# medvedevgroup/SibeliaZ

Hardware: AMD Instinct MI355X
Metric: seed vertices/sec through BlocksFinder (higher is better)
Workload: dtype int32

## Files before the change

### sibeliaz_amd/csrc/lcb_kernel.h

```cpp
#ifndef LCB_KERNEL_H
#define LCB_KERNEL_H

#include <hip/hip_runtime.h>
#include <stdint.h>

#include "lcb_kernel_limits.h"

#define LCB_EMPTY_KEY INT32_MIN
#if defined(__HIP_DEVICE_COMPILE__)
#define LCB_NO_LOADS_IN_FLIGHT() __builtin_amdgcn_s_waitcnt(0x0F70)
#else
#define LCB_NO_LOADS_IN_FLIGHT() ((void)0)
#endif
#if defined(__HIP_DEVICE_COMPILE__)
#define LCB_GLOBAL_U32(p) ((const __attribute__((address_space(1))) uint32_t*)(p))
#else
#define LCB_GLOBAL_U32(p) (p)
#endif
#ifndef LCB_PROF_PUSH
#define LCB_PROF_PUSH 0
#endif

template <int MODE> struct LcbCfg;
template <> struct LcbCfg<0> { static constexpr uint32_t IC = 256, VC = 1024, BW = 256, PC = 0; static constexpr bool INST_LDS = true, IDX_LDS = true; typedef uint16_t Idx; typedef uint32_t VLast; };
// ... 115 lines not shown

#define LCB_WAVE_SYNC_LDS()                                       \
    do {                                                          \
        __builtin_amdgcn_fence(__ATOMIC_RELEASE, "wavefront");    \
        __builtin_amdgcn_wave_barrier();                          \
        __builtin_amdgcn_fence(__ATOMIC_ACQUIRE, "wavefront");    \
    } while (0)
#define LCB_SYNC_IF(ldsResident) do { if (ldsResident) LCB_WAVE_SYNC_LDS(); else LCB_WAVE_SYNC(); } while (0)

#define LCB_MARK(S, slot, value)                                                         \
    do {                                                                                 \
        if ((S).dbg && (S).lane == 0) __hip_atomic_store(&(S).dbg[(slot)], (uint32_t)(value), __ATOMIC_RELAXED, __HIP_MEMORY_SCOPE_SYSTEM); \
    } while (0)

__device__ __forceinline__ uint32_t lcb_rfl(uint32_t v) { return (uint32_t)__builtin_amdgcn_readfirstlane((int)v); }
__device__ __forceinline__ int32_t lcb_rfl(int32_t v) { return __builtin_amdgcn_readfirstlane(v); }
__device__ __forceinline__ uint64_t lcb_rfl(uint64_t v) { return ((uint64_t)lcb_rfl((uint32_t)(v >> 32)) << 32) | lcb_rfl((uint32_t)v); }
__device__ __forceinline__ uint32_t lcb_rl(uint32_t v, uint32_t l) { return (uint32_t)__builtin_amdgcn_readlane((int)v, (int)l); }
__device__ __forceinline__ uint64_t lcb_rl(uint64_t v, uint32_t l) { return ((uint64_t)lcb_rl((uint32_t)(v >> 32), l) << 32) | lcb_rl((uint32_t)v, l); }
__device__ __forceinline__ int32_t lcb_rl(int32_t v, uint32_t l) { return __builtin_amdgcn_readlane(v, (int)l); }

__device__ __forceinline__ uint32_t lcb_wave_umax(uint32_t v)
{
    uint32_t t;
    t = (uint32_t)__builtin_amdgcn_update_dpp(0, (int)v, 0x111, 0xf, 0xf, false); v = v > t ? v : t;
    t = (uint32_t)__builtin_amdgcn_update_dpp(0, (int)v, 0x112, 0xf, 0xf, false); v = v > t ? v : t;
    t = (uint32_t)__builtin_amdgcn_update_dpp(0, (int)v, 0x114, 0xf, 0xf, false); v = v > t ? v : t;
    t = (uint32_t)__builtin_amdgcn_update_dpp(0, (int)v, 0x118, 0xf, 0xf, false); v = v > t ? v : t;
    t = (uint32_t)__builtin_amdgcn_update_dpp(0, (int)v, 0x142, 0xa, 0xf, false); v = v > t ? v : t;
    t = (uint32_t)__builtin_amdgcn_update_dpp(0, (int)v, 0x143, 0xc, 0xf, false); v = v > t ? v : t;
    return lcb_rl(v, 63);
}
__device__ __forceinline__ uint32_t lcb_wave_umin(uint32_t v) { return ~lcb_wave_umax(~v); }

#define LCB_FLAG_POS 1u
#define LCB_FLAG_BACKFIN 2u
#define LCB_FLAG_FRONTFIN 4u
#define LCB_FLAG_BITS 3u
#define LCB_FLAG_SEG_SHIFT (LCB_SEG_SHIFT + LCB_FLAG_BITS)

template <bool WIDE> struct LcbWidth { typedef uint32_t T; };
template <> struct LcbWidth<true> { typedef uint64_t T; };

template <int MODE_, bool SEG_>
struct LcbStateT {
    static constexpr int MODE = MODE_;
    typedef typename LcbCfg<MODE_>::Idx Idx;
    typedef typename LcbCfg<MODE_>::VLast VLast;
    static constexpr uint32_t NONE = (uint32_t)(Idx)~(Idx)0;
    static constexpr uint32_t LAST_SHIFT = 4u * sizeof(VLast);
    static constexpr bool SEG = SEG_;
    typedef typename LcbWidth<SEG_>::T Flat;
    typedef typename LcbWidth<SEG_>::T OccIdx;
    typedef uint32_t* FieldU;
    typedef int32_t* FieldI;
    LcbTables T;
    LcbUsed U;
    LcbKParams P;
    uint32_t lane;
    const uint64_t* segBase;
    uint32_t* segFirst;
    FieldU iFrontG, iBackG, iFrontPos, iBackPos, iLo, iHi, iFlags;
    FieldI iFrontDist, iBackDist;
    uint32_t* ordKey;
    Idx* ordIdx;
    Idx* good;
    Idx* goodPos;
    Idx* touch;
    uint32_t nTouch, nInit;
    uint32_t endInst;
    FieldU fpLo, fpHi;
    uint8_t* fpSeg8;
    uint32_t* fpSeg32;
    uint32_t nFp;
    uint32_t fpSplit, fpShift;
    uint32_t instCap;
    int32_t* vKey;
    uint32_t* vCount;
    VLast* vLast;
    Idx* vTouched;
    uint32_t* vNClaimed;
    uint32_t* vTicket;
    uint32_t* vOvf;
    uint32_t voteCap, voteShift;
    uint32_t* scr;
    uint32_t* bloom;
    uint32_t bloomShift;
    uint32_t* mail;
    uint32_t* part;
    unsigned long long* mailWalk;
    int32_t* pKeys;
    uint32_t* pSlots;
    uint32_t pathCap, pathShift;
    unsigned long long* body;
    uint32_t bodyCap;
    uint4* best;
    uint32_t bestCap;
    uint32_t* ck;
    uint32_t ckN, ckInst, ckGood, ckPath;
    int32_t ckFlank;
    uint32_t nInst, nGood, cur, nPath, nRight, nLeft, nBest, status;
    int32_t rightFlank, leftFlank;
    uint32_t* dbg;
    const uint32_t* abort;
    uint32_t pfPush, pfVote, pfMaxProbe, pfMaxInst;
    uint64_t pfTVote, pfTPush, pfTScore;
    uint64_t pfTWalk, pfTWaitB, pfTReduce, pfTScan;
    uint64_t pfVoters, pfChunks, pfTouchSum;
    uint64_t cWalk, cOcc, cCompatCall, cCompatStep, cVote, cPush;
};

#ifndef LCB_TEST_FP_SLOT_DIV
#define LCB_TEST_FP_SLOT_DIV 1u
#endif
template <class ST>
__device__ __forceinline__ uint32_t lcb_fp_slot(const ST& S, uint32_t i)
{
    if (i < S.fpSplit) return i;
    const uint32_t f = i + S.fpShift;
    return f < S.instCap / LCB_TEST_FP_SLOT_DIV ? f : i;
}

template <class ST>
__device__ __forceinline__ void lcb_fp_set_seg(ST& S, uint32_t fs, uint32_t seg)
{
    if (ST::SEG) { if (LcbCfg<ST::MODE>::INST_LDS) S.fpSeg8[fs] = (uint8_t)seg; else S.fpSeg32[fs] = seg; }
}
template <class ST>
__device__ __forceinline__ uint32_t lcb_fp_get_seg(const ST& S, uint32_t fs)
{
    return ST::SEG ? (LcbCfg<ST::MODE>::INST_LDS ? (uint32_t)S.fpSeg8[fs] : S.fpSeg32[fs]) : 0u;
}

enum { LCB_F_FRONTG = 0, LCB_F_BACKG, LCB_F_FRONTPOS, LCB_F_BACKPOS, LCB_F_LO, LCB_F_HI, LCB_F_FLAGS, LCB_F_FRONTDIST, LCB_F_BACKDIST, LCB_F_COUNT };
template <class ST>
__device__ __forceinline__ uint32_t lcb_inst_fields(const ST& S, uint32_t i)
{
    const uint32_t stride = (uint32_t)(S.iBackG - S.iFrontG);
    uint32_t f = 0;
    if (S.lane < (uint32_t)LCB_F_COUNT) f = S.iFrontG[S.lane * stride + i];
    return f;
}

__device__ __forceinline__ uint32_t lcb_hash(int32_t vid, uint32_t shift)
{
    return ((uint32_t)vid * 2654435761u) >> shift;
}

__device__ __forceinline__ LcbUsed lcb_used_of(const LcbTables& T, uint32_t view)
{
    LcbUsed U;
    U.live = T.used;
    U.tab = view ? T.viewTab + (size_t)view * T.nPages : nullptr;
    return U;
}

__device__ __forceinline__ uint32_t lcb_uword(const LcbUsed& U, uint32_t w)
{
    if (U.tab) w += LCB_GLOBAL_U32(U.tab)[w >> LCB_PAGE_SHIFT];
    return U.live[w];
}

template <class ST>
__device__ __forceinline__ typename ST::Flat lcb_seg_base(const ST& S, uint32_t seg) { return ST::SEG ? (typename ST::Flat)S.segBase[seg] : (typename ST::Flat)0; }
__device__ __forceinline__ uint32_t lcb_cw_seg(uint32_t cw) { return cw >> LCB_SEG_SHIFT; }
__device__ __forceinline__ uint32_t lcb_fl_seg(uint32_t fl) { return fl >> LCB_FLAG_SEG_SHIFT; }
// ... 477 lines not shown
                uint32_t first = 0;
#define LCB_SCAN64(x, base) if (!first && n > (base)) { const uint32_t c_ = n - (base) < 64u ? n - (base) : 64u; const uint64_t m_ = (x) & (c_ == 64u ? ~0ull : ((1ull << c_) - 1ull)); if (m_) first = (base) + (uint32_t)__ffsll((long long)m_); }
                LCB_SCAN64(x0, 0u) LCB_SCAN64(x1, 64u) LCB_SCAN64(x2, 128u) LCB_SCAN64(x3, 192u)
#undef LCB_SCAN64
                for (uint32_t d = have + 1; !first && d <= Lu; d++)
                    if (lcb_used_bit(S.U, (Flat)(up ? fb + (d - 1u) : fb - (d - 1u)))) first = d;
                if (first) { nv = first - 1u; brk = 1u; }
            }
        }
        if (isV && !tryUsed) {
            const uint32_t ge = up ? g0 + nv : g0 - nv;
            const uint32_t fs = lcb_fp_slot(S, vI);
            atomicMin(&S.fpLo[fs], ge);
            atomicMax(&S.fpHi[fs], ge);
        }
        if (STATS && isV) S.cWalk += nv + brk;
        auto consume = [&](uint32_t b, uint32_t c, int32_t id) {
            if (PROF) S.pfChunks++;
            const uint32_t bn = lcb_rl(nv, b), bf = lcb_rl(fl, b);
            const uint32_t d = c * 64 + S.lane + 1;
            bool act = d <= bn;
            const int32_t vid = (bf & LCB_FLAG_POS) ? id : -id;
            if (exact) {
                const unsigned long long hitM = __ballot(act && lcb_path_contains(S, vid));
                if (hitM) {
                    const uint32_t fh = (uint32_t)__ffsll((long long)hitM) - 1u;
                    act = act && S.lane < fh;
                    if (S.lane == b) {
                        const uint32_t nn = c * 64 + fh;
                        if (STATS) S.cWalk += (uint64_t)(nn + 1u) - (uint64_t)(nv + brk);
                        nv = nn; brk = 1u;
                    }
                }
            }
            const uint32_t wgt = lcb_rl(weight, b), e = lcb_rl(vE, b);
            if (act) {
                uint32_t h = lcb_hash(vid, S.voteShift);
                int32_t old = atomicCAS(&S.vKey[h], LCB_EMPTY_KEY, vid);
                uint32_t probe = 0;
                while (old != LCB_EMPTY_KEY && old != vid && probe < S.voteCap) {
                    h = (h + 1) & vmask; probe++;
                    old = atomicCAS(&S.vKey[h], LCB_EMPTY_KEY, vid);
                }
                if (old == LCB_EMPTY_KEY) {
                    const uint32_t tt = atomicAdd(S.vNClaimed, 1u);
                    if (tt < claimCap) S.vTouched[tt] = (typename ST::Idx)h; else *S.vOvf = 1u;
                }
                if (old == LCB_EMPTY_KEY || old == vid) {
                    atomicAdd(&S.vCount[h], wgt);
                    atomicMax(&S.vLast[h], ((typename ST::VLast)e << ST::LAST_SHIFT) | d);
                } else *S.vOvf = 1u;
            }
        };
        unsigned long long rest = walkM;
        uint32_t curB = 0, curC = 0, curN = 0, ord = 0;
        bool curOn = false;
        auto nextItem = [&](uint32_t& b, uint32_t& c) -> bool {
            for (;;) {
                if (curOn) {
                    curN = lcb_rl(nv, curB);
                    if (curC * 64 < curN) { b = curB; c = curC++; return true; }
                    curOn = false;
                }
                if (!rest) return false;
                curB = (uint32_t)__ffsll((long long)rest) - 1u; rest &= rest - 1;
                curC = ord < (uint32_t)LCB_VB ? 1u : 0u; ord++;
                curOn = true;
            }
        };
        for (;;) {
#pragma unroll
            for (int q = 0; q < LCB_VB; q++) if (itV[q]) consume(itB[q], itC[q], itId[q]);
#pragma unroll
            for (int q = 0; q < LCB_VB; q++) {
                itV[q] = nextItem(itB[q], itC[q]);
                itId[q] = 0;
                if (itV[q]) itId[q] = request(itB[q], itC[q]);
            }
            if (!itV[0]) break;
        }
    }
}

template <class ST>
__device__ inline bool lcb_vote_any_in_path(const ST& S, uint32_t s0, uint32_t s1)
{
    bool hit = false;
    for (uint32_t q = s0 + S.lane; q < s1; q += 64) if (lcb_path_contains(S, S.vKey[S.vTouched[q]])) hit = true;
    return __ballot(hit) != 0;
}

struct LcbBest { uint32_t cnt, keyHi, keyLo; int32_t vid; uint32_t e; };

template <class ST>
__device__ inline LcbBest lcb_vote_argmax(const ST& S, bool forward, bool useGood, uint32_t s0, uint32_t s1)
{
    uint32_t bCnt = 0, bHi = 0xFFFFFFFFu, bLo = 0xFFFFFFFFu, bE = 0;
    int32_t bVid = 0;
    for (uint32_t q = s0 + S.lane; q < s1; q += 64) {
        const uint32_t t = S.vTouched[q];
        const int32_t key = S.vKey[t];
        const uint32_t cnt = S.vCount[t];
        const typename ST::VLast last = S.vLast[t];
        const uint32_t e = (uint32_t)(last >> ST::LAST_SHIFT), d = (uint32_t)(last & (((typename ST::VLast)1 << ST::LAST_SHIFT) - 1));
        const uint32_t i = useGood ? S.good[e] : e;
        const uint32_t g0 = forward ? S.iBackG[i] : S.iFrontG[i];
        const uint32_t afl = S.iFlags[i];
        const uint32_t hi = ((afl & LCB_FLAG_POS) << 31) | (ST::SEG ? lcb_fl_seg(afl) << 26 : 0u) | (g0 >> 6), lo = (g0 << 26) | d;
        if (cnt > bCnt || (cnt == bCnt && (hi < bHi || (hi == bHi && lo < bLo)))) { bCnt = cnt; bHi = hi; bLo = lo; bVid = key; bE = e; }
    }
    LcbBest r;
    r.cnt = lcb_wave_umax(bCnt);
    bool c = bCnt == r.cnt && r.cnt != 0;
    r.keyHi = lcb_wave_umin(c ? bHi : 0xFFFFFFFFu);
    c = c && bHi == r.keyHi;
    r.keyLo = lcb_wave_umin(c ? bLo : 0xFFFFFFFFu);
    c = c && bLo == r.keyLo;
    const unsigned long long m = __ballot(c);
    const uint32_t w = m ? (uint32_t)__ffsll((long long)m) - 1u : 0u;
    r.vid = m ? lcb_rl(bVid, w) : 0;
    r.e = lcb_rl(bE, w);
    return r;
}

enum { LCB_MAIL_CMD = 0, LCB_MAIL_FLAGS, LCB_MAIL_NLIST, LCB_MAIL_FLANK, LCB_MAIL_NTOUCH, LCB_MAIL_FPSPLIT, LCB_MAIL_FPSHIFT, LCB_MAIL_WORDS = 8 };
enum { LCB_CMD_VOTE = 1, LCB_CMD_EXIT = 2 };

template <class ST>
__device__ inline void lcb_vote_clear(ST& S, uint32_t s0, uint32_t s1)
{
    for (uint32_t q = s0 + S.lane; q < s1; q += 64) { const uint32_t t = S.vTouched[q]; S.vKey[t] = LCB_EMPTY_KEY; S.vCount[t] = 0; S.vLast[t] = 0; }
}

#ifndef LCB_VOTE_SHARE_MIN
#define LCB_VOTE_SHARE_MIN 24u
#endif

template <int NW, class ST>
__device__ inline void lcb_vote_reduce_slice(ST& S, bool forward, bool useGood, uint32_t waveId, uint32_t nTouched, bool exact)
{
    const uint32_t per = (nTouched + NW - 1) / NW;
    const uint32_t s0 = waveId * per < nTouched ? waveId * per : nTouched, s1 = s0 + per < nTouched ? s0 + per : nTouched;
    const bool hit = !exact && lcb_vote_any_in_path(S, s0, s1);
    const LcbBest b = lcb_vote_argmax(S, forward, useGood, s0, s1);
    if (S.lane == 0) {
        uint32_t* p = S.part + 8 * waveId;
        p[0] = b.cnt; p[1] = b.keyHi; p[2] = b.keyLo; p[3] = (uint32_t)b.vid; p[4] = b.e; p[5] = hit ? 1u : 0u;
    }
    __syncthreads();
    lcb_vote_clear(S, s0, s1);
    __syncthreads();
}

template <bool STATS, int NW, bool PROF = false, class ST>
__device__ inline LcbBest lcb_vote_pass(ST& S, bool forward, bool tryUsed, bool useGood, bool exact, bool& ovfAny, bool& hit)
{
    const uint32_t claimCap = S.voteCap - (S.voteCap >> 2);
    LcbBest b;
    hit = false;
    const bool multi = NW > 1 && S.nTouch > 1;
    const bool share = multi && S.nTouch >= LCB_VOTE_SHARE_MIN;
    if (multi) {
        if (S.lane == 0) {
            S.mail[LCB_MAIL_FLAGS] = (forward ? 1u : 0u) | (tryUsed ? 2u : 0u) | (useGood ? 4u : 0u) | (share ? 8u : 0u) | (exact ? 16u : 0u);
            S.mail[LCB_MAIL_NTOUCH] = S.nTouch;
            S.mail[LCB_MAIL_FPSPLIT] = S.fpSplit; S.mail[LCB_MAIL_FPSHIFT] = S.fpShift;
            if (!LCB_WALK_V2_OF(ST)) *S.vTicket = 0;
            S.mail[LCB_MAIL_CMD] = LCB_CMD_VOTE;
        }
        __syncthreads();
    }
    const uint64_t tw0 = PROF ? wall_clock64() : 0;
    lcb_vote_walk<STATS, PROF>(S, forward, tryUsed, useGood, 0, multi ? (uint32_t)NW : 1u, exact);
    const uint64_t tw1 = PROF ? wall_clock64() : 0;
    if (multi) __syncthreads();
    else LCB_SYNC_IF(LcbCfg<ST::MODE>::IDX_LDS);
    const uint64_t tw2 = PROF ? wall_clock64() : 0;
    if (PROF && !LCB_PROF_PUSH) { S.pfTWalk += tw1 - tw0; S.pfTWaitB += tw2 - tw1; }
    uint32_t nTouched = lcb_rfl(*S.vNClaimed);
    if (nTouched > claimCap) nTouched = claimCap;
    if (STATS && multi && S.lane == 0) { S.cWalk += *S.mailWalk; *S.mailWalk = 0; }
    const uint32_t per = share ? (nTouched + NW - 1) / NW : nTouched;
    const uint32_t s1 = per < nTouched ? per : nTouched;
    hit = !exact && lcb_vote_any_in_path(S, 0, s1);
    b = lcb_vote_argmax(S, forward, useGood, 0, s1);
    if (share) {
        if (S.lane == 0) {
            uint32_t* p = S.part;
            p[0] = b.cnt; p[1] = b.keyHi; p[2] = b.keyLo; p[3] = (uint32_t)b.vid; p[4] = b.e; p[5] = hit ? 1u : 0u;
        }
        __syncthreads();
        lcb_vote_clear(S, 0, s1);
        __syncthreads();
        uint32_t pc = 0, ph = 0xFFFFFFFFu, pl = 0xFFFFFFFFu, pv = 0, pe = 0, pHit = 0;
        if (S.lane < (uint32_t)NW) { const uint32_t* p = S.part + 8 * S.lane; pc = p[0]; ph = p[1]; pl = p[2]; pv = p[3]; pe = p[4]; pHit = p[5]; }
        hit = __ballot(pHit != 0) != 0;
        b.cnt = lcb_wave_umax(pc);
        bool c = pc == b.cnt && b.cnt != 0;
        b.keyHi = lcb_wave_umin(c ? ph : 0xFFFFFFFFu); c = c && ph == b.keyHi;
        b.keyLo = lcb_wave_umin(c ? pl : 0xFFFFFFFFu); c = c && pl == b.keyLo;
        const unsigned long long m = __ballot(c);
        const uint32_t w = m ? (uint32_t)__ffsll((long long)m) - 1u : 0u;
        b.vid = m ? (int32_t)lcb_rl(pv, w) : 0;
        b.e = lcb_rl(pe, w);
    } else {
        LCB_SYNC_IF(LcbCfg<ST::MODE>::IDX_LDS);
        lcb_vote_clear(S, 0, s1);
    }
    if (PROF && !LCB_PROF_PUSH) S.pfTReduce += wall_clock64() - tw2;
    ovfAny = lcb_rfl(*S.vOvf) != 0;
    if (S.lane == 0) { *S.vNClaimed = 0; *S.vOvf = 0; }
    LCB_SYNC_IF(LcbCfg<ST::MODE>::IDX_LDS);
    return b;
}

template <bool STATS, bool PROF, int NW, class ST>
__device__ inline int32_t lcb_vote(ST& S, bool forward, uint32_t attempts, uint32_t& originInst)
{
    const bool useGood = S.nGood >= 2;
    const uint32_t nList = useGood ? S.nGood : S.nInst;
    originInst = 0;
    constexpr bool DEFER = LcbCfg<ST::MODE>::BW != 0;
    for (uint32_t attempt = 0; attempt < attempts; attempt++) {
        const bool tryUsed = attempt != 0;
        if (STATS && S.lane == 0) S.cVote++;
        if (PROF) S.pfVote++;
        if (nList == 0 || S.nTouch == 0) continue;
        const uint64_t cWalk0 = S.cWalk;
        bool ovfAny = false, hit = false;
        if (PROF) S.pfTouchSum += S.nTouch;
        LcbBest b;
        for (uint32_t pass = 0;; pass++) {
            b = lcb_vote_pass<STATS, NW, PROF>(S, forward, tryUsed, useGood, pass != 0 || !DEFER, ovfAny, hit);
            if (pass != 0 || !DEFER || !(hit || ovfAny)) break;
            if (ovfAny) {
                for (uint32_t h = S.lane; h < S.voteCap; h += 64) { S.vKey[h] = LCB_EMPTY_KEY; S.vCount[h] = 0; S.vLast[h] = 0; }
                LCB_SYNC_IF(LcbCfg<ST::MODE>::IDX_LDS);
            }
            if (STATS) S.cWalk = cWalk0;
            if (PROF) S.pfMaxProbe++;
        }
        if (ovfAny) { S.status = LCB_ST_VOTE_OVF; return 0; }
        if (b.cnt == 0) continue;
        originInst = useGood ? lcb_rfl((uint32_t)S.good[b.e]) : b.e;
        return b.vid;
    }
    return 0;
}

template <class F> struct LcbOccT { uint4 rec; uint32_t lo, hi, g0, uw0, uw1, uw2; F sb; };

template <class J>
__device__ __forceinline__ uint4 lcb_load_rec(const LcbTables& T, J j, bool active)
{
    uint4 r = uint4{0u, 0u, 0u, 0u};
    if (active) r = T.occRec[j];
    return r;
}

template <class ST>
__device__ __forceinline__ LcbOccT<typename ST::Flat> lcb_finish_occ(const ST& S, const uint4& rec, bool active)
{
    const LcbTables& T = S.T;
    const LcbUsed& U = S.U;
    typedef typename ST::Flat Flat;
    LcbOccT<Flat> o;
    o.rec = rec; o.lo = 0; o.hi = 0; o.g0 = 0; o.uw0 = o.uw1 = o.uw2 = 0; o.sb = 0;
    if (active) {
        const uint2 lh = T.chrLoHi[rec.y & LCB_CHR_MASK];
        o.lo = lh.x; o.hi = lh.y;
        o.sb = lcb_seg_base(S, lcb_cw_seg(rec.y));
        const Flat f = o.sb + rec.x;
        const uint32_t wi = (uint32_t)(f >> 5);
        const uint32_t wbase = wi ? wi - 1 : 0;
        o.g0 = rec.x - ((uint32_t)f & 31u) - (wi ? 32u : 0u);
        if (U.tab) {
            const uint32_t pg = wi >> LCB_PAGE_SHIFT, d = U.tab[pg];
            const uint32_t w1 = wbase + 1, w2 = wbase + 2;
            o.uw0 = U.live[wbase + ((wbase >> LCB_PAGE_SHIFT) == pg ? d : U.tab[wbase >> LCB_PAGE_SHIFT])];
            o.uw1 = U.live[w1 + ((w1 >> LCB_PAGE_SHIFT) == pg ? d : U.tab[w1 >> LCB_PAGE_SHIFT])];
            o.uw2 = U.live[w2 + ((w2 >> LCB_PAGE_SHIFT) == pg ? d : U.tab[w2 >> LCB_PAGE_SHIFT])];
        } else { o.uw0 = U.live[wbase]; o.uw1 = U.live[wbase + 1]; o.uw2 = U.live[wbase + 2]; }
    }
    return o;
}

template <class F>
__device__ __forceinline__ bool lcb_occ_bit(const LcbOccT<F>& o, uint32_t g)
{
    const uint32_t off = g - o.g0;
    const uint64_t lo = (uint64_t)o.uw0 | ((uint64_t)o.uw1 << 32);
    return off < 64u ? ((lo >> off) & 1ull) != 0 : ((o.uw2 >> (off - 64u)) & 1u) != 0;
}

template <class F>
__device__ __forceinline__ bool lcb_range_any_used_c(const LcbUsed& U, const LcbOccT<F>& o, uint32_t a, uint32_t b)
{
    if (a >= b) return false;
    const uint32_t oa = a - o.g0, ob = b - o.g0;
    if (oa >= 96u || ob > 96u || ob < oa) return lcb_range_any_used(U, (F)(o.sb + a), (F)(o.sb + b));
    const uint64_t lo = (uint64_t)o.uw0 | ((uint64_t)o.uw1 << 32);
    bool any = false;
    if (oa < 64u) {
        const uint32_t e = ob < 64u ? ob : 64u;
        const uint64_t m = (e == 64u ? ~0ull : ((1ull << e) - 1ull)) & ~((1ull << oa) - 1ull);
        any = (lo & m) != 0;
    }
    if (ob > 64u) {
        const uint32_t s = oa > 64u ? oa - 64u : 0u, e = ob - 64u;
        const uint32_t m = (e == 32u ? 0xFFFFFFFFu : ((1u << e) - 1u)) & ~((1u << s) - 1u);
        any = any || (o.uw2 & m) != 0;
    }
    return any;
}

template <class J> struct LcbEdgeT { uint32_t gIt, segIt; bool itPositive; int32_t idIt, idN; uint32_t posIt, posN; int32_t ech; J o0; uint32_t nOcc; };

// ... 451 lines not shown
            lcb_path_init<STATS>(S, vid, ch);
        }
        while (from < nEdge && !S.status) {
            const uint32_t nE = nEdge - from < 64 ? nEdge - from : 64;
            LcbEdgeBatchT<typename ST::OccIdx> bt;
            lcb_batch_from_body(S, from, nE, bt);
            uint4 rec = lcb_load_rec(S.T, lcb_rl(bt.o0, 0) + S.lane, S.lane < lcb_rl(bt.nOcc, 0));
            for (uint32_t l = 0; l < nE && !S.status; l++) {
                const LcbEdgeT<typename ST::OccIdx> E = lcb_edge_of(bt, l);
                uint4 recN = uint4{0u, 0u, 0u, 0u};
                if (l + 1 < nE) recN = lcb_load_rec(S.T, lcb_rl(bt.o0, l + 1) + S.lane, S.lane < lcb_rl(bt.nOcc, l + 1));
                lcb_push<true, STATS, PROF>(S, E, false, rec);
                rec = recN;
            }
            from += nE;
        }
        if (!S.status && bestScore > 0) lcb_snapshot(S);
        S.fpSplit = S.nInst; S.fpShift = S.nFp - S.nInst;
    }
    LCB_MARK(S, 2, 4);
    if (!S.status && !dead) {
        for (uint32_t i = S.lane; i < S.nInit; i += 64) S.touch[i] = (typename ST::Idx)i;
        S.nTouch = S.nInit;
        LCB_WAVE_SYNC();
        for (;;) {
            bool ret = true;
            const int64_t prevLength = (int64_t)S.rightFlank - S.leftFlank;
            while ((ret = lcb_extend<false, STATS, PROF, NW>(S, bestRightSize, bestScore, score)) &&
                   ((int64_t)S.rightFlank - S.leftFlank) - prevLength <= minRun)
                ;
            const bool positive = score > 0;
            if (!ret || !positive || S.status) break;
        }
    }
    LCB_MARK(S, 2, 5);
    S.endInst = S.nInst;
    lcb_path_clear(S);
    bestScoreOut = bestScore;
}

struct LcbLaunchArgs {
    const LcbKSeed* seeds;
    LcbSeedOut* out;
    LcbSeedCtr* ctr;
    uint4* arena;
    LcbFpOut* fpArena;
    unsigned long long arenaCap, fpCap, arenaBase, fpBase;
    unsigned long long* arenaCursor;
    unsigned long long* fpCursor;
    uint32_t* cursor;
    const uint32_t* live;
    uint32_t cursorBase, nSeeds;
    const uint32_t* usedTab;
};

template <int MODE, bool STATS, int NW, bool PROF, bool SEG = false>
__device__ inline void lcb_process_body(const LcbTables& T, const LcbKParams& P, const LcbKSeed* seeds, uint32_t nSeeds,
                                        const LcbWork& W, LcbSeedOut* out, uint4* arena, unsigned long long arenaCap,
                                        LcbFpOut* fpArena, unsigned long long fpCap)
{
    typedef LcbCfg<MODE> Cfg;
    constexpr bool INST_LDS = Cfg::INST_LDS, IDX_LDS = Cfg::IDX_LDS;
    constexpr uint32_t IC = Cfg::IC, VC = Cfg::VC, BW = Cfg::BW, PC = Cfg::PC;
    __shared__ uint32_t sInst[INST_LDS ? 9 * IC : 1];
    __shared__ uint32_t sFp[INST_LDS ? 2 * IC : 1];
    __shared__ uint32_t sOrdKey[IDX_LDS ? 2 * IC : 1];
    typedef typename Cfg::Idx Idx;
    typedef typename Cfg::VLast VLast;
    __shared__ Idx sOrdIdx[IDX_LDS ? 2 * IC : 1];
    __shared__ Idx sGood[IDX_LDS ? IC : 1];
    __shared__ Idx sGoodPos[IDX_LDS ? IC : 1];
    __shared__ Idx sTouch[IDX_LDS ? IC : 1];
    __shared__ int32_t sVKey[IDX_LDS ? VC : 1];
    __shared__ uint32_t sVCount[IDX_LDS ? VC : 1];
    __shared__ VLast sVLast[IDX_LDS ? VC : 1];
    __shared__ Idx sVTouched[IDX_LDS ? VC : 1];
    __shared__ uint32_t sBloom[BW ? BW : 1];
    __shared__ int32_t sPath[PC ? PC : 1];
    __shared__ uint32_t sScr[(SEG ? 4 : 3) * 64];
    __shared__ uint64_t sSegBase[SEG ? LCB_MAX_SEG : 1];
    __shared__ uint32_t sSegFirst[SEG ? LCB_MAX_SEG + 2 : 1];
    __shared__ uint8_t sFpSeg[(SEG && INST_LDS) ? IC : 1];
    __shared__ uint32_t sMisc[4];
    __shared__ uint32_t sMail[LCB_MAIL_WORDS];
    __shared__ uint32_t sPart[8 * NW];
    __shared__ unsigned long long sMailWalk[1];
    __shared__ LcbLaunchArgs sArgs;
    if (threadIdx.x == 0) {
        sArgs.seeds = seeds; sArgs.out = out; sArgs.ctr = W.ctr; sArgs.arena = arena; sArgs.fpArena = fpArena; sArgs.arenaCap = arenaCap; sArgs.fpCap = fpCap;
        sArgs.arenaBase = W.arenaBase; sArgs.fpBase = W.fpBase; sArgs.arenaCursor = W.arenaCursor; sArgs.fpCursor = W.fpCursor;
        sArgs.cursor = W.cursor; sArgs.cursorBase = W.cursorBase; sArgs.live = W.live; sArgs.nSeeds = W.live ? *W.nLive : nSeeds;
    }

    LcbStateT<MODE, SEG> S;
    S.T = T; S.P = P; S.U = lcb_used_of(T, 0);
    S.lane = threadIdx.x & 63u;
    S.segBase = sSegBase; S.segFirst = sSegFirst;
    if (SEG) {
        if (threadIdx.x < LCB_MAX_SEG) sSegBase[threadIdx.x] = threadIdx.x < T.nSeg ? T.segBase[threadIdx.x] : 0ull;
        if (threadIdx.x < LCB_MAX_SEG + 2) sSegFirst[threadIdx.x] = 0;
    }
    uint8_t* slot = W.base + (uint64_t)blockIdx.x * W.slotBytes;
    const LcbSlotLayout L = lcb_slot_layout(W.pathCap, W.bodyCap, W.bestCap, INST_LDS ? 0 : W.instCap, IDX_LDS ? 0 : W.voteCap);
    S.pSlots = (uint32_t*)(slot + L.pSlots);
    if (PC) { S.pKeys = sPath; S.pathCap = W.pathCap < PC ? W.pathCap : PC; for (uint32_t h = threadIdx.x; h < PC; h += 64 * NW) sPath[h] = LCB_EMPTY_KEY; }
    else { S.pKeys = (int32_t*)(slot + L.pKeys); S.pathCap = W.pathCap; }
    S.pathShift = 32u - (uint32_t)__ffs((int)S.pathCap) + 1u;
    S.body = (unsigned long long*)(slot + L.body); S.bodyCap = W.bodyCap;
    S.best = (uint4*)(slot + L.best); S.bestCap = W.bestCap;
    S.ck = (uint32_t*)(slot + L.ck); S.ckN = S.ckInst = S.ckGood = S.ckPath = 0; S.ckFlank = 0;
    uint32_t* instBase;
    uint32_t instStride;
    uint32_t *fpBase;
    if (INST_LDS) { instBase = sInst; instStride = IC; fpBase = sFp; }
    else { instBase = (uint32_t*)(slot + L.inst); instStride = W.instCap; fpBase = (uint32_t*)(slot + L.fp); }
    S.fpLo = fpBase; S.fpHi = fpBase + instStride;
    S.fpSeg8 = sFpSeg; S.fpSeg32 = INST_LDS ? nullptr : fpBase + 2 * instStride;
    if (IDX_LDS) {
        S.instCap = IC;
        S.ordKey = sOrdKey; S.ordIdx = sOrdIdx; S.good = sGood; S.goodPos = sGoodPos; S.touch = sTouch;
        S.vKey = sVKey; S.vCount = sVCount; S.vLast = sVLast; S.vTouched = sVTouched;
        S.voteCap = VC;
        for (uint32_t h = threadIdx.x; h < VC; h += 64 * NW) { sVKey[h] = LCB_EMPTY_KEY; sVCount[h] = 0; sVLast[h] = 0; }
    } else {
        S.instCap = W.instCap;
        S.ordKey = (uint32_t*)(slot + L.ordKey); S.ordIdx = (Idx*)(slot + L.ordIdx);
        S.good = (Idx*)(slot + L.good); S.goodPos = (Idx*)(slot + L.goodPos); S.touch = (Idx*)(slot + L.touch);
        S.vKey = (int32_t*)(slot + L.vKey); S.vCount = (uint32_t*)(slot + L.vCount);
        S.vLast = (VLast*)(slot + L.vLast); S.vTouched = (Idx*)(slot + L.vTouched);
        S.voteCap = W.voteCap;
    }
    S.bloom = sBloom;
    S.bloomShift = BW ? 32u - (uint32_t)__ffs((int)(BW * 32u)) + 1u : 0u;
    for (uint32_t h = threadIdx.x; h < BW; h += 64 * NW) sBloom[h] = 0;
    S.voteShift = 32u - (uint32_t)__ffs((int)S.voteCap) + 1u;
    S.iFrontG = instBase; S.iBackG = instBase + instStride;
    S.iFrontPos = instBase + 2 * instStride; S.iBackPos = instBase + 3 * instStride;
    S.iLo = instBase + 4 * instStride; S.iHi = instBase + 5 * instStride;
    S.iFlags = instBase + 6 * instStride;
    S.iFrontDist = (int32_t*)(instBase + 7 * instStride);
    S.iBackDist = (int32_t*)(instBase + 8 * instStride);
    S.scr = sScr; S.vNClaimed = &sMisc[0]; S.vOvf = &sMisc[1]; S.vTicket = &sMisc[2];
    S.mail = sMail; S.mailWalk = sMailWalk; S.part = sPart;
    const uint32_t waveId = lcb_rfl(threadIdx.x >> 6);
    S.dbg = (W.dbg && waveId == 0) ? W.dbg + 16u * blockIdx.x : nullptr;
    S.abort = W.abort;
    LCB_MARK(S, 0, 1);
    if (threadIdx.x == 0) { sMisc[0] = 0; sMisc[1] = 0; sMisc[2] = 0; sMail[LCB_MAIL_CMD] = 0; sMailWalk[0] = 0; }
    S.nInst = S.nGood = S.cur = S.nPath = S.nRight = S.nLeft = S.nBest = 0; S.status = 0; S.nTouch = S.nInit = 0;
    S.rightFlank = S.leftFlank = 0;
    S.cWalk = S.cOcc = S.cCompatCall = S.cCompatStep = S.cVote = S.cPush = 0;
    S.pfPush = S.pfVote = S.pfMaxProbe = S.pfMaxInst = 0; S.pfTVote = S.pfTPush = S.pfTScore = 0; S.nFp = 0;
    S.pfTWalk = S.pfTWaitB = S.pfTReduce = S.pfTScan = 0; S.pfVoters = S.pfChunks = S.pfTouchSum = 0;
    LCB_WAVE_SYNC();
    if (NW > 1) {
        __syncthreads();
        if (waveId != 0) {
            for (;;) {
                __syncthreads();
                if (lcb_rfl(S.mail[LCB_MAIL_CMD]) == LCB_CMD_EXIT) return;
                S.U.tab = sArgs.usedTab;
                const uint32_t flags = lcb_rfl(S.mail[LCB_MAIL_FLAGS]);
                S.nTouch = lcb_rfl(S.mail[LCB_MAIL_NTOUCH]);
                S.fpSplit = lcb_rfl(S.mail[LCB_MAIL_FPSPLIT]); S.fpShift = lcb_rfl(S.mail[LCB_MAIL_FPSHIFT]);
                S.cWalk = 0;
                lcb_vote_walk<STATS>(S, (flags & 1u) != 0, (flags & 2u) != 0, (flags & 4u) != 0, waveId, NW, (flags & 16u) != 0);
                if (STATS) {
                    const unsigned long long w = (unsigned long long)lcb_wave_sum((int64_t)S.cWalk);
                    if (S.lane == 0 && w) atomicAdd(S.mailWalk, w);
                }
                __syncthreads();
                if (flags & 8u) {
                    uint32_t nTouched = lcb_rfl(*S.vNClaimed);
                    const uint32_t claimCap = S.voteCap - (S.voteCap >> 2);
                    if (nTouched > claimCap) nTouched = claimCap;
                    lcb_vote_reduce_slice<NW>(S, (flags & 1u) != 0, (flags & 4u) != 0, waveId, nTouched, (flags & 16u) != 0);
                }
            }
        }
    } else LCB_WAVE_SYNC();

    for (;;) {
        uint32_t tk = 0;
        if (S.lane == 0) tk = atomicAdd(sArgs.cursor, 1u) - sArgs.cursorBase;
        tk = lcb_rfl(tk);
        if (tk >= sArgs.nSeeds) break;
        const uint32_t s = sArgs.live ? lcb_rfl(sArgs.live[tk]) : tk;
        LCB_MARK(S, 1, s + 1);
        S.cWalk = S.cOcc = S.cCompatCall = S.cCompatStep = S.cVote = S.cPush = 0;
        S.nInst = S.nGood = S.cur = S.nRight = S.nLeft = 0; S.rightFlank = S.leftFlank = 0;
        S.nFp = 0;
        int64_t bestScore = 0;
        S.pfPush = S.pfVote = S.pfMaxProbe = S.pfMaxInst = 0; S.pfTVote = S.pfTPush = S.pfTScore = 0;
        S.pfTWalk = S.pfTWaitB = S.pfTReduce = S.pfTScan = 0; S.pfVoters = S.pfChunks = S.pfTouchSum = 0;
        const uint64_t tick0 = PROF ? wall_clock64() : 0;
        const LcbKSeed sd = sArgs.seeds[s];
        const int32_t vid = lcb_rfl(sd.vid), ch = lcb_rfl(sd.ch);
        S.U = lcb_used_of(T, lcb_rfl(sd.view));
        if (NW > 1 && S.lane == 0) sArgs.usedTab = S.U.tab;
        lcb_process_seed<MODE, STATS, PROF, NW>(S, vid, ch, bestScore);
        if (S.status == LCB_ST_VOTE_OVF) {
            LCB_WAVE_SYNC();
            for (uint32_t h = S.lane; h < S.voteCap; h += 64) { S.vKey[h] = LCB_EMPTY_KEY; S.vCount[h] = 0; S.vLast[h] = 0; }
            if (S.lane == 0) { *S.vNClaimed = 0; *S.vOvf = 0; }
            LCB_WAVE_SYNC();
        }
        const uint64_t ticks = PROF ? wall_clock64() - tick0 : 0;
        const uint32_t n = S.status ? 0u : S.nBest;
        unsigned long long off = 0;
        if (n) {
            uint32_t olo = 0, ohi = 0;
            if (S.lane == 0) { off = atomicAdd(sArgs.arenaCursor, (unsigned long long)n) - sArgs.arenaBase; olo = (uint32_t)off; ohi = (uint32_t)(off >> 32); }
            olo = lcb_rfl(olo); ohi = lcb_rfl(ohi);
            off = ((unsigned long long)ohi << 32) | olo;
            if (off + n > sArgs.arenaCap) S.status = LCB_ST_ARENA_OVF;
            else { uint4* ar = sArgs.arena; for (uint32_t e = S.lane; e < n; e += 64) ar[off + e] = S.best[e]; }
        }
        LcbFpOut* fpa = sArgs.fpArena;
        const uint32_t nfp = (S.status == LCB_ST_OK && fpa) ? S.nFp : 0u;
        unsigned long long fpo = 0;
        if (nfp) {
            uint32_t olo = 0, ohi = 0;
            if (S.lane == 0) { fpo = atomicAdd(sArgs.fpCursor, (unsigned long long)nfp) - sArgs.fpBase; olo = (uint32_t)fpo; ohi = (uint32_t)(fpo >> 32); }
            olo = lcb_rfl(olo); ohi = lcb_rfl(ohi);
            fpo = ((unsigned long long)ohi << 32) | olo;
            if (fpo + nfp > sArgs.fpCap) S.status = LCB_ST_ARENA_OVF;
            else for (uint32_t e = S.lane; e < nfp; e += 64) {
#ifdef LCB_TEST_PLAIN_FP_READ
                const uint32_t lo = S.fpLo[e], hi = S.fpHi[e];
#else
                const uint32_t lo = INST_LDS ? S.fpLo[e] : __hip_atomic_load(&S.fpLo[e], __ATOMIC_RELAXED, __HIP_MEMORY_SCOPE_AGENT);
                const uint32_t hi = INST_LDS ? S.fpHi[e] : __hip_atomic_load(&S.fpHi[e], __ATOMIC_RELAXED, __HIP_MEMORY_SCOPE_AGENT);
#endif
                const uint64_t sb = lcb_seg_base(S, lcb_fp_get_seg(S, e));
                LcbFpOut r; r.lo = sb + (lo ? lo - 1 : 0u); r.hi = sb + hi; fpa[fpo + e] = r;
            }
        }
        uint64_t c0 = 0, c1 = 0, c2 = 0, c3 = 0, c4 = 0, c5 = 0;
        if (STATS) {
            c0 = (uint64_t)lcb_wave_sum((int64_t)S.cWalk); c1 = (uint64_t)lcb_wave_sum((int64_t)S.cOcc);
            c2 = (uint64_t)lcb_wave_sum((int64_t)S.cCompatCall); c3 = (uint64_t)lcb_wave_sum((int64_t)S.cCompatStep);
            c4 = (uint64_t)lcb_wave_sum((int64_t)S.cVote); c5 = (uint64_t)lcb_wave_sum((int64_t)S.cPush);
        }
        if (S.lane == 0) {
            LcbSeedOut* o = sArgs.out + s;
            o->nInst = n;
            o->bestScore = bestScore; o->arenaOff = off;
            o->fpOff = fpo; o->nFp = nfp; o->poolInst = S.endInst;
        }
// ... 55 lines not shown
```

Baseline: 926,900.

## Resolve voter walk lengths on leader wave, then distribute vote chunks across waves

```diff
diff --git a/sibeliaz_amd/csrc/lcb_kernel.h b/sibeliaz_amd/csrc/lcb_kernel.h
--- a/sibeliaz_amd/csrc/lcb_kernel.h
+++ b/sibeliaz_amd/csrc/lcb_kernel.h
@@ -221,6 +221,8 @@
     uint32_t* vNClaimed;
     uint32_t* vTicket;
     uint32_t* vOvf;
+    uint32_t* vRec;
+    uint32_t* vItem;
     uint32_t voteCap, voteShift;
     uint32_t* scr;
     uint32_t* bloom;
@@ -864,6 +866,233 @@
     }
 }
 
+template <class F> struct LcbVoterReq {
+    bool isV, walks, scan, positive, up;
+    uint32_t vI, vE, g0, rem, weight, fl, win;
+    F fb;
+    uint32_t uw0, uw1, uw2, uw3, uw4, uw5, uw6, uw7;
+};
+template <class ST>
+__device__ __forceinline__ LcbVoterReq<typename ST::Flat> lcb_voter_request(const ST& S, uint32_t t, uint32_t nTouch, bool forward, bool tryUsed, bool useGood, uint32_t maxW)
+{
+    const LcbTables& T = S.T;
+    typedef typename ST::Flat Flat;
+    LcbVoterReq<Flat> R;
+    R.isV = false;
+    R.vI = 0; R.vE = 0; R.g0 = 0; R.rem = 0; R.weight = 0; R.fl = 0;
+    if (t < nTouch) {
+        R.vI = S.touch[t];
+        R.vE = useGood ? (uint32_t)S.goodPos[R.vI] : R.vI;
+        R.isV = R.vE != ST::NONE;
+    }
+    if (R.isV) {
+        R.fl = S.iFlags[R.vI];
+        const uint32_t fp = S.iFrontPos[R.vI], bp = S.iBackPos[R.vI];
+        R.g0 = forward ? S.iBackG[R.vI] : S.iFrontG[R.vI];
+        const uint32_t lo = S.iLo[R.vI], hi = S.iHi[R.vI];
+        R.weight = lcb_absdiff(fp, bp) + 1u;
+        R.rem = (forward == ((R.fl & LCB_FLAG_POS) != 0)) ? hi - 1u - R.g0 : R.g0 - lo;
+    }
+    R.positive = (R.fl & LCB_FLAG_POS) != 0; R.up = forward == R.positive;
+    Flat sb = 0;
+    if (ST::SEG) sb = (Flat)S.segBase[lcb_fl_seg(R.fl)];
+    const Flat f0 = sb + R.g0;
+    R.walks = R.isV && R.rem != 0;
+    R.win = 0;
+    if (R.walks) R.win = T.posWin[f0];
+    const uint32_t delta = R.positive ? 0u : 1u;
+    R.scan = R.walks && !tryUsed && !(!R.up && f0 < (Flat)(1u + delta));
+    R.fb = R.scan ? (R.up ? f0 + 1u - delta : f0 - 1u - delta) : (Flat)0;
+    R.uw0 = 0; R.uw1 = 0; R.uw2 = 0; R.uw3 = 0; R.uw4 = 0; R.uw5 = 0; R.uw6 = 0; R.uw7 = 0;
+    if (R.scan) {
+        const uint32_t W0 = (uint32_t)(R.fb >> 5);
+        const uint32_t um = R.up ? 0xFFFFFFFFu : 0u;
+#define LCB_WIDX(k) ((((W0 + (k)) < maxW ? (W0 + (k)) : maxW) & um) | ((W0 - (W0 < (k) ? W0 : (k))) & ~um))
+        uint32_t a0 = LCB_WIDX(0u), a1 = LCB_WIDX(1u), a2 = LCB_WIDX(2u), a3 = LCB_WIDX(3u), a4 = LCB_WIDX(4u), a5 = LCB_WIDX(5u), a6 = LCB_WIDX(6u), a7 = LCB_WIDX(7u);
+#undef LCB_WIDX
+        if (S.U.tab) {
+            const auto tab = LCB_GLOBAL_U32(S.U.tab);
+            const uint32_t o0 = tab[a0 >> LCB_PAGE_SHIFT], o1 = tab[a1 >> LCB_PAGE_SHIFT], o2 = tab[a2 >> LCB_PAGE_SHIFT], o3 = tab[a3 >> LCB_PAGE_SHIFT];
+            const uint32_t o4 = tab[a4 >> LCB_PAGE_SHIFT], o5 = tab[a5 >> LCB_PAGE_SHIFT], o6 = tab[a6 >> LCB_PAGE_SHIFT], o7 = tab[a7 >> LCB_PAGE_SHIFT];
+            a0 += o0; a1 += o1; a2 += o2; a3 += o3; a4 += o4; a5 += o5; a6 += o6; a7 += o7;
+        }
+        R.uw0 = S.U.live[a0]; R.uw1 = S.U.live[a1]; R.uw2 = S.U.live[a2]; R.uw3 = S.U.live[a3];
+        R.uw4 = S.U.live[a4]; R.uw5 = S.U.live[a5]; R.uw6 = S.U.live[a6]; R.uw7 = S.U.live[a7];
+    }
+    return R;
+}
+
+template <bool STATS, class ST>
+__device__ __forceinline__ void lcb_voter_resolve(ST& S, LcbVoterReq<typename ST::Flat>& R, uint32_t dm, bool tryUsed, uint32_t& nv, uint32_t& brk)
+{
+    typedef typename ST::Flat Flat;
+    nv = 0; brk = 0;
+    if (R.walks) {
+        const uint32_t wv = R.up ? (R.win & 0xFFFFu) : (R.win >> 16);
+        uint32_t L = wv > dm ? wv : dm;
+        if (L > R.rem) L = R.rem;
+        nv = L;
+        if (R.scan) {
+            const bool up = R.up;
+            const Flat fb = R.fb;
+            uint32_t uw0 = R.uw0, uw1 = R.uw1, uw2 = R.uw2, uw3 = R.uw3, uw4 = R.uw4, uw5 = R.uw5, uw6 = R.uw6, uw7 = R.uw7;
+            const uint32_t Lu = (!R.positive && !up && L == R.rem) ? L - 1u : L;
+            const uint32_t sh = up ? ((uint32_t)fb & 31u) : 31u - ((uint32_t)fb & 31u);
+            if (!up) { uw0 = LCB_BREV32(uw0); uw1 = LCB_BREV32(uw1); uw2 = LCB_BREV32(uw2); uw3 = LCB_BREV32(uw3); uw4 = LCB_BREV32(uw4); uw5 = LCB_BREV32(uw5); uw6 = LCB_BREV32(uw6); uw7 = LCB_BREV32(uw7); }
+            const uint64_t s0 = (uint64_t)uw0 | ((uint64_t)uw1 << 32), s1 = (uint64_t)uw2 | ((uint64_t)uw3 << 32), s2 = (uint64_t)uw4 | ((uint64_t)uw5 << 32), s3 = (uint64_t)uw6 | ((uint64_t)uw7 << 32);
+            const uint64_t x0 = (s0 >> sh) | ((s1 << 1) << (63u - sh)), x1 = (s1 >> sh) | ((s2 << 1) << (63u - sh)), x2 = (s2 >> sh) | ((s3 << 1) << (63u - sh)), x3 = s3 >> sh;
+            const uint32_t have = 256u - sh;
+            const uint32_t n = Lu < have ? Lu : have;
+            uint32_t first = 0;
+#define LCB_SCAN64(x, base) if (!first && n > (base)) { const uint32_t c_ = n - (base) < 64u ? n - (base) : 64u; const uint64_t m_ = (x) & (c_ == 64u ? ~0ull : ((1ull << c_) - 1ull)); if (m_) first = (base) + (uint32_t)__ffsll((long long)m_); }
+            LCB_SCAN64(x0, 0u) LCB_SCAN64(x1, 64u) LCB_SCAN64(x2, 128u) LCB_SCAN64(x3, 192u)
+#undef LCB_SCAN64
+            for (uint32_t d = have + 1; !first && d <= Lu; d++)
+                if (lcb_used_bit(S.U, (Flat)(up ? fb + (d - 1u) : fb - (d - 1u)))) first = d;
+            if (first) { nv = first - 1u; brk = 1u; }
+        }
+    }
+    if (R.isV && !tryUsed) {
+        const uint32_t ge = R.up ? R.g0 + nv : R.g0 - nv;
+        const uint32_t fs = lcb_fp_slot(S, R.vI);
+        atomicMin(&S.fpLo[fs], ge);
+        atomicMax(&S.fpHi[fs], ge);
+    }
+    if (STATS && R.isV) S.cWalk += nv + brk;
+}
+
+#ifndef LCB_VOTE_RESOLVE_MODES
+#define LCB_VOTE_RESOLVE_MODES 0x6u
+#endif
+#ifndef LCB_VOTE_RESOLVE_MIN
+#define LCB_VOTE_RESOLVE_MIN 24u
+#endif
+#ifndef LCB_VOTE_RESOLVE_MAX
+#define LCB_VOTE_RESOLVE_MAX 256u
+#endif
+#ifndef LCB_VOTE_RESOLVE_ITEMS
+#define LCB_VOTE_RESOLVE_ITEMS 2048u
+#endif
+#define LCB_VOTE_RESOLVE_OF(MODE, NW) ((NW) > 2 && ((MODE) == 1 || (MODE) == 2) && (((LCB_VOTE_RESOLVE_MODES) >> (MODE)) & 1u) != 0)
+static_assert(LCB_VOTE_RESOLVE_MIN >= 2u && LCB_VOTE_RESOLVE_MAX <= 65536u, "a resolved vote wakes the helpers; a record index has 16 bits");
+enum { LCB_RV_RESOLVED = 0, LCB_RV_CHUNK1, LCB_RV_USED_BEYOND_64, LCB_RV_REPEAT_HIT, LCB_RV_ABOVE_MAX, LCB_RV_ITEMS_FULL, LCB_RV_ROUND2, LCB_RV_COUNT };
+#ifdef LCB_TEST_RESOLVE_EVENT
+void LCB_TEST_RESOLVE_EVENT(int what);
+#define LCB_RESOLVE_EVENT_IF(cond, what) do { if (cond) LCB_TEST_RESOLVE_EVENT(what); } while (0)
+#else
+#define LCB_RESOLVE_EVENT_IF(cond, what) ((void)0)
+#endif
+#define LCB_RESOLVE_EVENT(S, what) LCB_RESOLVE_EVENT_IF((S).lane == 0, what)
+
+template <int NW, class ST>
+__device__ __forceinline__ bool lcb_vote_resolves(const ST& S)
+{
+    return LCB_VOTE_RESOLVE_OF(ST::MODE, NW) && S.nTouch >= LCB_VOTE_RESOLVE_MIN && S.nTouch <= LCB_VOTE_RESOLVE_MAX;
+}
+
+__device__ __forceinline__ uint32_t lcb_wave_scan(uint32_t v)
+{
+    v += (uint32_t)__builtin_amdgcn_update_dpp(0, (int)v, 0x111, 0xf, 0xf, false);
+    v += (uint32_t)__builtin_amdgcn_update_dpp(0, (int)v, 0x112, 0xf, 0xf, false);
+    v += (uint32_t)__builtin_amdgcn_update_dpp(0, (int)v, 0x114, 0xf, 0xf, false);
+    v += (uint32_t)__builtin_amdgcn_update_dpp(0, (int)v, 0x118, 0xf, 0xf, false);
+    v += (uint32_t)__builtin_amdgcn_update_dpp(0, (int)v, 0x142, 0xa, 0xf, false);
+    v += (uint32_t)__builtin_amdgcn_update_dpp(0, (int)v, 0x143, 0xc, 0xf, false);
+    return v;
+}
+
+template <bool STATS, bool PROF, class ST>
+__device__ inline uint32_t lcb_vote_resolve(ST& S, bool forward, bool tryUsed, bool useGood)
+{
+    typedef typename ST::Flat Flat;
+    const uint32_t depth = (uint32_t)S.P.depth;
+    const uint32_t dm = depth ? depth - 1u : 0u;
+    const uint32_t nTouch = S.nTouch;
+    const uint32_t maxW = (uint32_t)(S.T.nPos >> 5);
+    uint32_t nRec = 0, nItems = 0;
+    for (uint32_t p0 = 0; p0 < nTouch; p0 += 64) {
+        LCB_NO_LOADS_IN_FLIGHT();
+        LcbVoterReq<Flat> R = lcb_voter_request(S, p0 + S.lane, nTouch, forward, tryUsed, useGood, maxW);
+        uint32_t nv, brk;
+        lcb_voter_resolve<STATS>(S, R, dm, tryUsed, nv, brk);
+        if (PROF) S.pfVoters += (uint32_t)__popcll(__ballot(R.walks));
+        LCB_RESOLVE_EVENT_IF(brk && nv >= 64u, LCB_RV_USED_BEYOND_64);
+        const bool has = nv != 0;
+        const unsigned long long hasM = __ballot(has);
+        const uint32_t nch = (nv + 63u) >> 6;
+        const uint32_t incl = lcb_wave_scan(nch);
+        const uint32_t total = lcb_rl(incl, 63);
+        if (nItems + total > LCB_VOTE_RESOLVE_ITEMS) return ~0u;
+        if (has) {
+            const uint32_t r = nRec + (uint32_t)__popcll(hasM & ((1ull << S.lane) - 1));
+            uint32_t* rec = S.vRec + 4u * r;
+            rec[0] = R.g0; rec[1] = nv | (R.positive ? 0x10000u : 0u) | (lcb_fl_seg(R.fl) << 17); rec[2] = R.weight; rec[3] = R.vE;
+            uint32_t* it = S.vItem + nItems + (incl - nch);
+            for (uint32_t c = 0; c < nch; c++) it[c] = r | (c << 16);
+        }
+        nRec += (uint32_t)__popcll(hasM); nItems += total;
+    }
+    return nItems;
+}
+
+template <bool PROF, class ST>
+__device__ inline void lcb_vote_items(ST& S, bool forward, uint32_t nItems)
+{
+    const LcbTables& T = S.T;
+    typedef typename ST::Flat Flat;
+    const uint32_t vmask = S.voteCap - 1;
+    const uint32_t claimCap = S.voteCap - (S.voteCap >> 2);
+    for (;;) {
+        uint32_t t = 0;
+        if (S.lane == 0) t = atomicAdd(S.vTicket, (uint32_t)LCB_VB);
+        t = lcb_rfl(t);
+        if (t >= nItems) break;
+        uint32_t itF[LCB_VB], itC[LCB_VB];
+        int32_t itId[LCB_VB];
+#pragma unroll
+        for (int q = 0; q < LCB_VB; q++) {
+            itF[q] = 0; itC[q] = 0; itId[q] = 0;
+            if (t + q < nItems) {
+                const uint32_t it = lcb_rfl(S.vItem[t + q]);
+                itC[q] = it >> 16;
+                if (S.lane < 4u) itF[q] = S.vRec[4u * (it & 0xFFFFu) + S.lane];
+                const uint32_t g0 = lcb_rl(itF[q], 0), w1 = lcb_rl(itF[q], 1);
+                const bool up = forward == ((w1 & 0x10000u) != 0);
+                const uint32_t d = itC[q] * 64 + S.lane + 1;
+                const Flat sb = ST::SEG ? (Flat)lcb_rfl(S.segBase[w1 >> 17]) : (Flat)0;
+                if (d <= (w1 & 0xFFFFu)) itId[q] = (T.posId + sb)[up ? g0 + d : g0 - d];
+            }
+        }
+#pragma unroll
+        for (int q = 0; q < LCB_VB; q++) {
+            if (t + q < nItems) {
+                if (PROF) S.pfChunks++;
+                if (itC[q]) LCB_RESOLVE_EVENT(S, LCB_RV_CHUNK1);
+                const uint32_t w1 = lcb_rl(itF[q], 1), wgt = lcb_rl(itF[q], 2), e = lcb_rl(itF[q], 3);
+                const uint32_t d = itC[q] * 64 + S.lane + 1;
+                const int32_t vid = (w1 & 0x10000u) ? itId[q] : -itId[q];
+                if (d <= (w1 & 0xFFFFu)) {
+                    uint32_t h = lcb_hash(vid, S.voteShift);
+                    int32_t old = atomicCAS(&S.vKey[h], LCB_EMPTY_KEY, vid);
+                    uint32_t probe = 0;
+                    while (old != LCB_EMPTY_KEY && old != vid && probe < S.voteCap) {
+                        h = (h + 1) & vmask; probe++;
+                        old = atomicCAS(&S.vKey[h], LCB_EMPTY_KEY, vid);
+                    }
+                    if (old == LCB_EMPTY_KEY) {
+                        const uint32_t tt = atomicAdd(S.vNClaimed, 1u);
+                        if (tt < claimCap) S.vTouched[tt] = (typename ST::Idx)h; else *S.vOvf = 1u;
+                    }
+                    if (old == LCB_EMPTY_KEY || old == vid) {
+                        atomicAdd(&S.vCount[h], wgt);
+                        atomicMax(&S.vLast[h], ((typename ST::VLast)e << ST::LAST_SHIFT) | d);
+                    } else *S.vOvf = 1u;
+                }
+            }
+        }
+    }
+}
+
 template <class ST>
 __device__ inline bool lcb_vote_any_in_path(const ST& S, uint32_t s0, uint32_t s1)
 {
@@ -905,7 +1134,7 @@
     return r;
 }
 
-enum { LCB_MAIL_CMD = 0, LCB_MAIL_FLAGS, LCB_MAIL_NLIST, LCB_MAIL_FLANK, LCB_MAIL_NTOUCH, LCB_MAIL_FPSPLIT, LCB_MAIL_FPSHIFT, LCB_MAIL_WORDS = 8 };
+enum { LCB_MAIL_CMD = 0, LCB_MAIL_FLAGS, LCB_MAIL_NLIST, LCB_MAIL_FLANK, LCB_MAIL_NTOUCH, LCB_MAIL_FPSPLIT, LCB_MAIL_FPSHIFT, LCB_MAIL_NITEMS, LCB_MAIL_WORDS = 8 };
 enum { LCB_CMD_VOTE = 1, LCB_CMD_EXIT = 2 };
 
 template <class ST>
@@ -942,23 +1171,39 @@
     hit = false;
     const bool multi = NW > 1 && S.nTouch > 1;
     const bool share = multi && S.nTouch >= LCB_VOTE_SHARE_MIN;
+    bool resolve = !exact && lcb_vote_resolves<NW>(S);
+    uint32_t nItems = 0;
+    uint64_t tResolve = 0;
+    if (LCB_VOTE_RESOLVE_OF(ST::MODE, NW) && resolve) {
+        const uint64_t tr0 = PROF ? wall_clock64() : 0;
+        const uint64_t cWalk0 = S.cWalk;
+        nItems = lcb_vote_resolve<STATS, PROF>(S, forward, tryUsed, useGood);
+        if (nItems == ~0u) {
+            resolve = false; nItems = 0;
+            if (STATS) S.cWalk = cWalk0;
+            LCB_RESOLVE_EVENT(S, LCB_RV_ITEMS_FULL);
+        } else { LCB_RESOLVE_EVENT(S, LCB_RV_RESOLVED); LCB_RESOLVE_EVENT_IF(S.lane == 0 && S.nTouch > 64u, LCB_RV_ROUND2); }
+        if (PROF) tResolve = wall_clock64() - tr0;
+    }
     if (multi) {
         if (S.lane == 0) {
-            S.mail[LCB_MAIL_FLAGS] = (forward ? 1u : 0u) | (tryUsed ? 2u : 0u) | (useGood ? 4u : 0u) | (share ? 8u : 0u) | (exact ? 16u : 0u);
+            S.mail[LCB_MAIL_FLAGS] = (forward ? 1u : 0u) | (tryUsed ? 2u : 0u) | (useGood ? 4u : 0u) | (share ? 8u : 0u) | (exact ? 16u : 0u) | (resolve ? 32u : 0u);
             S.mail[LCB_MAIL_NTOUCH] = S.nTouch;
             S.mail[LCB_MAIL_FPSPLIT] = S.fpSplit; S.mail[LCB_MAIL_FPSHIFT] = S.fpShift;
-            if (!LCB_WALK_V2_OF(ST)) *S.vTicket = 0;
+            S.mail[LCB_MAIL_NITEMS] = nItems;
+            if (!LCB_WALK_V2_OF(ST) || resolve) *S.vTicket = 0;
             S.mail[LCB_MAIL_CMD] = LCB_CMD_VOTE;
         }
         __syncthreads();
     }
     const uint64_t tw0 = PROF ? wall_clock64() : 0;
-    lcb_vote_walk<STATS, PROF>(S, forward, tryUsed, useGood, 0, multi ? (uint32_t)NW : 1u, exact);
+    if (LCB_VOTE_RESOLVE_OF(ST::MODE, NW) && resolve) lcb_vote_items<PROF>(S, forward, nItems);
+    else lcb_vote_walk<STATS, PROF>(S, forward, tryUsed, useGood, 0, multi ? (uint32_t)NW : 1u, exact);
     const uint64_t tw1 = PROF ? wall_clock64() : 0;
     if (multi) __syncthreads();
     else LCB_SYNC_IF(LcbCfg<ST::MODE>::IDX_LDS);
     const uint64_t tw2 = PROF ? wall_clock64() : 0;
-    if (PROF && !LCB_PROF_PUSH) { S.pfTWalk += tw1 - tw0; S.pfTWaitB += tw2 - tw1; }
+    if (PROF && !LCB_PROF_PUSH) { S.pfTWalk += tw1 - tw0 + tResolve; S.pfTWaitB += tw2 - tw1; }
     uint32_t nTouched = lcb_rfl(*S.vNClaimed);
     if (nTouched > claimCap) nTouched = claimCap;
     if (STATS && multi && S.lane == 0) { S.cWalk += *S.mailWalk; *S.mailWalk = 0; }
@@ -1012,9 +1257,12 @@
         bool ovfAny = false, hit = false;
         if (PROF) S.pfTouchSum += S.nTouch;
         LcbBest b;
+        const bool defer = DEFER || lcb_vote_resolves<NW>(S);
+        LCB_RESOLVE_EVENT_IF(S.lane == 0 && LCB_VOTE_RESOLVE_OF(ST::MODE, NW) && S.nTouch > LCB_VOTE_RESOLVE_MAX, LCB_RV_ABOVE_MAX);
         for (uint32_t pass = 0;; pass++) {
-            b = lcb_vote_pass<STATS, NW, PROF>(S, forward, tryUsed, useGood, pass != 0 || !DEFER, ovfAny, hit);
-            if (pass != 0 || !DEFER || !(hit || ovfAny)) break;
+            b = lcb_vote_pass<STATS, NW, PROF>(S, forward, tryUsed, useGood, pass != 0 || !defer, ovfAny, hit);
+            if (pass != 0 || !defer || !(hit || ovfAny)) break;
+            LCB_RESOLVE_EVENT_IF(S.lane == 0 && hit && lcb_vote_resolves<NW>(S), LCB_RV_REPEAT_HIT);
             if (ovfAny) {
                 for (uint32_t h = S.lane; h < S.voteCap; h += 64) { S.vKey[h] = LCB_EMPTY_KEY; S.vCount[h] = 0; S.vLast[h] = 0; }
                 LCB_SYNC_IF(LcbCfg<ST::MODE>::IDX_LDS);
@@ -1632,6 +1880,9 @@
     __shared__ uint32_t sSegFirst[SEG ? LCB_MAX_SEG + 2 : 1];
     __shared__ uint8_t sFpSeg[(SEG && INST_LDS) ? IC : 1];
     __shared__ uint32_t sMisc[4];
+    constexpr bool RESOLVE = LCB_VOTE_RESOLVE_OF(MODE, NW);
+    __shared__ uint32_t sVRec[RESOLVE ? 4 * LCB_VOTE_RESOLVE_MAX : 1];
+    __shared__ uint32_t sVItem[RESOLVE ? LCB_VOTE_RESOLVE_ITEMS : 1];
     __shared__ uint32_t sMail[LCB_MAIL_WORDS];
     __shared__ uint32_t sPart[8 * NW];
     __shared__ unsigned long long sMailWalk[1];
@@ -1692,6 +1943,7 @@
     S.iBackDist = (int32_t*)(instBase + 8 * instStride);
     S.scr = sScr; S.vNClaimed = &sMisc[0]; S.vOvf = &sMisc[1]; S.vTicket = &sMisc[2];
     S.mail = sMail; S.mailWalk = sMailWalk; S.part = sPart;
+    if (RESOLVE) { S.vRec = sVRec; S.vItem = sVItem; } else { S.vRec = nullptr; S.vItem = nullptr; }
     const uint32_t waveId = lcb_rfl(threadIdx.x >> 6);
     S.dbg = (W.dbg && waveId == 0) ? W.dbg + 16u * blockIdx.x : nullptr;
     S.abort = W.abort;
@@ -1714,7 +1966,8 @@
                 S.nTouch = lcb_rfl(S.mail[LCB_MAIL_NTOUCH]);
                 S.fpSplit = lcb_rfl(S.mail[LCB_MAIL_FPSPLIT]); S.fpShift = lcb_rfl(S.mail[LCB_MAIL_FPSHIFT]);
                 S.cWalk = 0;
-                lcb_vote_walk<STATS>(S, (flags & 1u) != 0, (flags & 2u) != 0, (flags & 4u) != 0, waveId, NW, (flags & 16u) != 0);
+                if (RESOLVE && (flags & 32u)) lcb_vote_items<false>(S, (flags & 1u) != 0, lcb_rfl(S.mail[LCB_MAIL_NITEMS]));
+                else lcb_vote_walk<STATS>(S, (flags & 1u) != 0, (flags & 2u) != 0, (flags & 4u) != 0, waveId, NW, (flags & 16u) != 0);
                 if (STATS) {
                     const unsigned long long w = (unsigned long long)lcb_wave_sum((int64_t)S.cWalk);
                     if (S.lane == 0 && w) atomicAdd(S.mailWalk, w);
```

Result: faster. 961,400 (median of 6 runs) (+3.7%).
